# andyburke/bitflood

Hardware: AMD Instinct MI355X
Metric: GiB/s device-resident chunk hashing, 256 KiB chunks, at 1/2/4/8 MI355X (higher is better)
Workload: dtype u32

## Files before the change

### bitflood_amd/_capi.py

```python
from __future__ import annotations

import ctypes
import os
import re

try:
    import torch
except Exception:
    torch = None

_HERE = os.path.dirname(os.path.abspath(__file__))
_REPO = os.path.dirname(_HERE)
LIB_PATH = os.environ.get("LBF_LIB") or os.path.join(_HERE, "lib", "liblbfhash.so")
HEADER_PATH = os.path.join(_REPO, "include", "lbf_hash.h")

LBF_OK = 0
LBF_ERR_INVALID = -1
LBF_ERR_NO_DEVICE = -2
LBF_ERR_HIP = -3
LBF_ERR_NOMEM = -4
LBF_ERR_IO = -5
LBF_HOST_PTR = 0
LBF_DEVICE_PTR = 1

_u8p = ctypes.POINTER(ctypes.c_uint8)
_c = ctypes
_SIGS = {
    "lbf_abi_version": (_c.c_int, []),
    "lbf_last_error": (_c.c_char_p, []),
    "lbf_device_count": (_c.c_int, [_c.POINTER(_c.c_int)]),
    "lbf_ctx_create": (_c.c_int, [_c.c_uint32, _c.POINTER(_c.c_void_p)]),
    "lbf_ctx_destroy": (None, [_c.c_void_p]),
    "lbf_ctx_num_devices": (_c.c_int, [_c.c_void_p]),
    "lbf_ctx_num_workers": (_c.c_int, [_c.c_void_p]),
    "lbf_ctx_worker_info": (_c.c_int, [_c.c_void_p, _c.c_int, _c.POINTER(_c.c_int), _c.POINTER(_c.c_int),
                                       _c.POINTER(_c.c_int), _c.POINTER(_c.c_int)]),
    "lbf_sha1_batch": (_c.c_int, [_c.c_void_p, _c.c_void_p, _c.c_uint64, _c.c_void_p, _c.c_void_p,
                                  _c.c_uint64, _c.c_void_p, _c.c_int]),
    "lbf_verify_batch": (_c.c_int, [_c.c_void_p, _c.c_void_p, _c.c_uint64, _c.c_void_p, _c.c_void_p,
                                    _c.c_uint64, _c.c_void_p, _c.c_void_p, _c.c_int]),
    "lbf_host_register": (_c.c_int, [_c.c_void_p, _c.c_void_p, _c.c_uint64]),
    "lbf_host_unregister": (_c.c_int, [_c.c_void_p, _c.c_void_p]),
    "lbf_ctx_staging_stats": (_c.c_int, [_c.c_void_p, _c.POINTER(_c.c_uint64), _c.POINTER(_c.c_uint64)]),
    "lbf_ctx_b64_stats": (_c.c_int, [_c.c_void_p, _c.POINTER(_c.c_uint64), _c.POINTER(_c.c_uint64)]),
    "lbf_sha1_one": (_c.c_int, [_c.c_void_p, _c.c_void_p, _c.c_uint32, _c.c_void_p]),
    "lbf_verify_encode_b64_batch": (_c.c_int, [_c.c_void_p, _c.c_void_p, _c.c_uint64, _c.c_void_p, _c.c_void_p,
                                               _c.c_uint64, _c.c_void_p, _c.c_void_p, _c.c_void_p, _c.c_uint64,
                                               _c.c_void_p]),
    "lbf_b64_put_length": (_c.c_uint64, [_c.c_uint64]),
    "lbf_b64_verify_batch": (_c.c_int, [_c.c_void_p, _c.c_void_p, _c.c_uint64, _c.c_void_p, _c.c_void_p,
                                        _c.c_uint64, _c.c_void_p, _c.c_void_p, _c.c_void_p, _c.c_uint64,
                                        _c.c_void_p, _c.c_void_p, _c.c_void_p]),
    "lbf_file_ranges": (_c.c_int, [_c.c_void_p, _c.c_char_p, _c.c_void_p, _c.c_void_p, _c.c_uint64,
                                   _c.c_void_p, _c.c_void_p]),
    "lbf_files_ranges": (_c.c_int, [_c.c_void_p, _c.c_void_p, _c.c_uint32, _c.c_void_p, _c.c_void_p, _c.c_void_p,
                                    _c.c_uint64, _c.c_void_p, _c.c_void_p]),
    "lbf_b64_27": (None, [_c.c_void_p, _c.c_char_p]),
    "lbf_b64_27_decode": (_c.c_int, [_c.c_char_p, _c.c_size_t, _c.c_void_p]),
    "lbf_sha1_launch": (_c.c_int, [_c.c_void_p, _c.c_void_p, _c.c_void_p, _c.c_uint64, _c.c_void_p,
                                   _c.c_void_p, _c.c_void_p, _c.c_void_p]),
    "lbf_sha1_uniform_launch": (_c.c_int, [_c.c_void_p, _c.c_uint64, _c.c_uint32, _c.c_uint64,
                                           _c.c_uint64, _c.c_void_p, _c.c_void_p, _c.c_void_p,
                                           _c.c_void_p]),
    "lbf_sha1_state_init": (None, [_c.c_void_p, _c.c_uint64]),
    "lbf_sha1_update_launch": (_c.c_int, [_c.c_void_p, _c.c_uint64, _c.c_void_p, _c.c_void_p, _c.c_void_p,
                                          _c.c_void_p, _c.c_void_p, _c.c_uint64, _c.c_void_p, _c.c_void_p,
                                          _c.c_void_p, _c.c_void_p]),
    "lbf_sha1_update_batch": (_c.c_int, [_c.c_void_p, _c.c_void_p, _c.c_uint64, _c.c_void_p, _c.c_void_p,
                                         _c.c_uint64, _c.c_void_p, _c.c_void_p, _c.c_void_p, _c.c_uint64,
                                         _c.c_void_p, _c.c_void_p, _c.c_void_p]),
    "lbf_b64_state_init": (None, [_c.c_void_p, _c.c_uint64]),
    "lbf_b64_update_launch": (_c.c_int, [_c.c_void_p, _c.c_void_p, _c.c_uint64, _c.c_void_p, _c.c_void_p, _c.c_void_p,
                                         _c.c_void_p, _c.c_void_p, _c.c_uint64, _c.c_void_p, _c.c_void_p, _c.c_void_p,
                                         _c.c_void_p, _c.c_void_p, _c.c_void_p, _c.c_void_p, _c.c_void_p, _c.c_void_p,
                                         _c.c_void_p]),
    "lbf_b64_update_batch": (_c.c_int, [_c.c_void_p, _c.c_void_p, _c.c_void_p, _c.c_uint64, _c.c_void_p, _c.c_void_p,
                                        _c.c_uint64, _c.c_void_p, _c.c_void_p, _c.c_void_p, _c.c_uint64, _c.c_void_p,
                                        _c.c_void_p, _c.c_void_p, _c.c_uint64, _c.c_void_p, _c.c_void_p, _c.c_void_p]),
    "lbf_set_kernel_variant": (_c.c_int, [_c.c_int]),
    "lbf_get_kernel_variant": (_c.c_int, []),
    "lbf_kernel_for": (_c.c_int, [_c.c_uint64]),
    "lbf_fill_synthetic": (_c.c_int, [_c.c_void_p, _c.c_uint64, _c.c_uint64, _c.c_uint64, _c.c_void_p]),
    "lbf_dev_malloc": (_c.c_int, [_c.POINTER(_c.c_void_p), _c.c_uint64]),
    "lbf_dev_free": (_c.c_int, [_c.c_void_p]),
    "lbf_memcpy_h2d": (_c.c_int, [_c.c_void_p, _c.c_void_p, _c.c_uint64]),
    "lbf_memcpy_d2h": (_c.c_int, [_c.c_void_p, _c.c_void_p, _c.c_uint64]),
    "lbf_set_device": (_c.c_int, [_c.c_int]),
    "lbf_device_synchronize": (_c.c_int, []),
    "lbf_stream_create": (_c.c_int, [_c.POINTER(_c.c_void_p)]),
    "lbf_stream_destroy": (_c.c_int, [_c.c_void_p]),
    "lbf_stream_synchronize": (_c.c_int, [_c.c_void_p]),
    "lbf_time_uniform": (_c.c_int, [_c.c_void_p, _c.c_uint64, _c.c_uint32, _c.c_uint64, _c.c_uint64,
                                    _c.c_void_p, _c.c_int, _c.c_void_p, _c.POINTER(_c.c_float)]),
}

_lib = None


class LbfError(RuntimeError):
    def __init__(self, status: int, msg: str):
        super().__init__(f"lbf status {status}: {msg}")
        self.status = status


def header_symbols(path: str = HEADER_PATH) -> list[str]:
    text = open(path).read()
    text = re.sub(r"/\*.*?\*/", "", text, flags=re.S)
    return sorted(set(re.findall(r"\b(lbf_[a-z0-9_]+)\s*\(", text)))


def load() -> ctypes.CDLL:
    global _lib
    if _lib is not None:
        return _lib
    if not os.path.exists(LIB_PATH):
        raise LbfError(LBF_ERR_INVALID,
                       f"{LIB_PATH} is not built; run `python -c 'import __graft_entry__ as g; g.build()'`")
    lib = ctypes.CDLL(LIB_PATH)
    for name, (res, args) in _SIGS.items():
        try:
            fn = getattr(lib, name)
        except AttributeError:
            if "LBF_LIB" in os.environ:
                continue
            raise
        fn.restype = res
        fn.argtypes = args
    _lib = lib
    return lib


def check(rc: int) -> None:
    if rc != LBF_OK:
        msg = load().lbf_last_error()
        raise LbfError(rc, msg.decode() if msg else "")


def device_count() -> int:
    n = ctypes.c_int(0)
    check(load().lbf_device_count(ctypes.byref(n)))
    return n.value
```

### bitflood_amd/csrc/lbf_internal.hpp

```cpp
#pragma once

#include <hip/hip_runtime.h>
#include <stdint.h>

#include <string>

#include "lbf_hash.h"

namespace lbf {

void set_error(const std::string& msg);
int fail(int status, const std::string& msg);
int hip_fail(hipError_t e, const char* what);

#define LBF_HIP_TRY(expr)                                   \
  do {                                                      \
    hipError_t lbf_e_ = (expr);                             \
    if (lbf_e_ != hipSuccess) return ::lbf::hip_fail(lbf_e_, #expr); \
  } while (0)

struct ChunkParams {
  const uint8_t* base;
  const uint64_t* offsets;
  const uint32_t* sizes;
  uint64_t len;
  uint64_t first_chunk;
  uint32_t chunk_size;
  uint32_t n;
  uint8_t* digests;
  const uint8_t* expected;
  uint8_t* verdicts;
};

int check_fits(const void* p, uint64_t bytes, const char* what);

int pick_variant(uint64_t n);
int launch_chunks(const ChunkParams& p, hipStream_t stream);

struct B64Launch {
  const uint8_t* text;
  uint8_t* scratch;
  const uint64_t* text_off;
  const uint64_t* sext_off;
  const uint32_t* text_len;
  uint8_t* out;
  const uint64_t* out_off;
  const uint32_t* cap;
  uint32_t* sizes;
  uint8_t* over;
  uint8_t* redo;
  uint32_t n;
  uint32_t max_text_len;
  uint32_t max_cap;
};
int launch_b64_decode(const B64Launch& b, hipStream_t stream);
int launch_b64_encode(const uint8_t* data, const uint64_t* data_off, const uint32_t* size, uint8_t* text,
                      const uint64_t* text_off, uint32_t n, uint32_t max_size, hipStream_t stream);

struct ExtraVariants {
  bool (*known)(int variant);
  bool (*launch)(int variant, const ChunkParams& p, hipStream_t stream);
};
extern const ExtraVariants* g_extra_variants;

}
```

### bitflood_amd/csrc/sha1_update.hip

```cpp
#include <hip/hip_runtime.h>
#include <stddef.h>

#include "lbf_internal.hpp"
#include "sha1_device.hpp"

namespace lbf {

namespace {

struct UpdateParams {
  uint8_t* states;
  uint64_t n_states;
  const uint32_t* state_of;
  const uint8_t* base;
  const uint64_t* offsets;
  const uint32_t* sizes;
  const uint8_t* final_flags;
  uint32_t n;
  uint8_t* digests;
  const uint8_t* expected;
  uint8_t* verdicts;
};

constexpr uint32_t kStateBytes = 96, kBlockAt = 32;
static_assert(sizeof(lbf_sha1_state) == kStateBytes, "lbf_sha1_state is 96 bytes");
static_assert(offsetof(lbf_sha1_state, buffered) == 20 && offsetof(lbf_sha1_state, total) == 24 &&
                  offsetof(lbf_sha1_state, block) == kBlockAt,
              "lbf_sha1_state layout");

__device__ __forceinline__ void load_block(uint4 (&q)[4], const uint4* src) {
  q[0] = src[0];
  q[1] = src[1];
  q[2] = src[2];
  q[3] = src[3];
}

__device__ __forceinline__ void update_blocks_aligned(Digest& s, const uint8_t* src, uint32_t nblk) {
  if (nblk == 0) return;
  const uint4* q = reinterpret_cast<const uint4*>(src);
  const uint32_t last = nblk - 1;
  uint4 A[4], B[4];
  load_block(A, q);
  load_block(B, q + 4 * (last < 1u ? last : 1u));
  for (uint32_t b = 0; b < nblk; ++b) {
    uint4 C[4] = {A[0], A[1], A[2], A[3]};
    A[0] = B[0]; A[1] = B[1]; A[2] = B[2]; A[3] = B[3];
    const uint32_t nb = b + 2 < last ? b + 2 : last;
    load_block(B, q + 4 * nb);
    uint32_t w[16];
    block_from_vec(w, C[0], C[1], C[2], C[3]);
    compress(s, w);
  }
}

__device__ __forceinline__ void update_blocks_unaligned(Digest& s, const uint8_t* src, uint32_t nblk) {
  for (uint32_t b = 0; b < nblk; ++b) {
    uint32_t w[16];
    load_words_any(w, src + 64ull * b, 64);
#pragma unroll
    for (int k = 0; k < 16; ++k) w[k] = bswap(w[k]);
    compress(s, w);
  }
}

__device__ __forceinline__ void record_block(uint32_t (&w)[16], const uint8_t* blk) {
  const uint4* q = reinterpret_cast<const uint4*>(blk);
  const uint4 q0 = q[0], q1 = q[1], q2 = q[2], q3 = q[3];
  block_from_vec(w, q0, q1, q2, q3);
}

__device__ __forceinline__ void finish64(Digest& s, uint32_t (&w)[16], uint32_t r, uint64_t total) {
#pragma unroll
  for (int k = 0; k < 16; ++k) {
    const int rem = (int)r - 4 * k;
    uint32_t v = w[k];
    if (rem <= 0) v = 0;
    if (rem >= 0 && rem < 4) {
      const uint32_t sh = 8u * (uint32_t)rem;
      v = (v & ~(0xFFFFFFFFu >> sh)) | (0x80000000u >> sh);
    }
    w[k] = v;
  }
  if (r >= 56) {
    compress(s, w);
#pragma unroll
    for (int k = 0; k < 16; ++k) w[k] = 0;
  }
  w[14] = (uint32_t)(total >> 29);
  w[15] = (uint32_t)(total << 3);
  compress(s, w);
}

__global__ void __launch_bounds__(256) sha1_update_kernel(UpdateParams p) {
  const uint32_t i = blockIdx.x * blockDim.x + threadIdx.x;
  if (i >= p.n) return;
  const uint64_t si = p.state_of ? (uint64_t)p.state_of[i] : (uint64_t)i;
  if (si >= p.n_states) return;
  uint8_t* const rec = p.states + kStateBytes * si;
  uint8_t* const blk = rec + kBlockAt;

  const uint4 lo = reinterpret_cast<const uint4*>(rec)[0];
  const uint4 hi = reinterpret_cast<const uint4*>(rec)[1];
  Digest s;
  s.h[0] = lo.x; s.h[1] = lo.y; s.h[2] = lo.z; s.h[3] = lo.w; s.h[4] = hi.x;
  uint32_t buf = hi.y & 63u;
  uint64_t total = (uint64_t)hi.z | ((uint64_t)hi.w << 32);

  const uint8_t* src = p.base + p.offsets[i];
  uint32_t size = p.sizes[i];
  const bool fin = p.final_flags != nullptr && p.final_flags[i] != 0;
  total += size;

  if (buf) {
    const uint32_t room = 64u - buf;
    const uint32_t take = size < room ? size : room;
    for (uint32_t k = 0; k < take; ++k) blk[(buf + k) & 63u] = src[k];
    src += take;
    size -= take;
    buf += take;
    if (buf == 64u) {
      uint32_t w[16];
      record_block(w, blk);
      compress(s, w);
      buf = 0;
    }
  }
  const uint32_t nblk = size >> 6;
  if ((reinterpret_cast<uintptr_t>(src) & 15u) == 0) {
    update_blocks_aligned(s, src, nblk);
  } else {
    update_blocks_unaligned(s, src, nblk);
  }
  src += 64ull * nblk;
  const uint32_t rem = size & 63u;
  for (uint32_t k = 0; k < rem; ++k) blk[(buf + k) & 63u] = src[k];
  buf = (buf + rem) & 63u;

  uint4* const out = reinterpret_cast<uint4*>(rec);
  if (!fin) {
    out[0] = make_uint4(s.h[0], s.h[1], s.h[2], s.h[3]);
    out[1] = make_uint4(s.h[4], buf, (uint32_t)total, (uint32_t)(total >> 32));
    return;
  }

  uint32_t w[16];
  record_block(w, blk);
  finish64(s, w, buf, total);
  uint32_t be[5];
#pragma unroll
  for (int k = 0; k < 5; ++k) be[k] = bswap(s.h[k]);
  if (p.digests) {
    uint32_t* o = reinterpret_cast<uint32_t*>(p.digests + 20ull * i);
#pragma unroll
    for (int k = 0; k < 5; ++k) o[k] = be[k];
  }
  if (p.verdicts) {
    const uint32_t* e = reinterpret_cast<const uint32_t*>(p.expected + 20ull * i);
    uint32_t diff = 0;
#pragma unroll
    for (int k = 0; k < 5; ++k) diff |= be[k] ^ e[k];
    p.verdicts[i] = diff == 0 ? 1 : 0;
  }
  out[0] = make_uint4(kH0, kH1, kH2, kH3);
  out[1] = make_uint4(kH4, 0u, 0u, 0u);
#pragma unroll
  for (int k = 2; k < 6; ++k) out[k] = make_uint4(0u, 0u, 0u, 0u);
}

}

}

using lbf::check_fits;
using lbf::fail;

extern "C" void lbf_sha1_state_init(lbf_sha1_state* states, uint64_t n) {
  if (!states) return;
  for (uint64_t k = 0; k < n; ++k) {
    lbf_sha1_state& s = states[k];
    s.h[0] = lbf::kH0; s.h[1] = lbf::kH1; s.h[2] = lbf::kH2; s.h[3] = lbf::kH3; s.h[4] = lbf::kH4;
    s.buffered = 0;
    s.total = 0;
    for (int j = 0; j < 64; ++j) s.block[j] = 0;
  }
}

extern "C" int lbf_sha1_update_launch(lbf_sha1_state* d_states, uint64_t n_states, const uint32_t* d_state_of,
                                      const uint8_t* d_base, const uint64_t* d_offsets, const uint32_t* d_sizes,
                                      const uint8_t* d_final, uint64_t n, uint8_t* d_digests,
                                      const uint8_t* d_expected, uint8_t* d_verdicts, void* stream) {
  const char* who = "lbf_sha1_update_launch";
  if (n == 0) return LBF_OK;
  if (!d_states || !d_base || !d_offsets || !d_sizes) return fail(LBF_ERR_INVALID, std::string(who) + ": null input");
  if (n > 0xFFFFFFFFull) return fail(LBF_ERR_INVALID, std::string(who) + ": n exceeds 2^32-1 per launch");
  if (d_final && !d_digests && !d_verdicts) return fail(LBF_ERR_INVALID, std::string(who) + ": no output");
  if ((d_verdicts != nullptr) != (d_expected != nullptr))
    return fail(LBF_ERR_INVALID, std::string(who) + ": expected and verdicts go together");
  if ((reinterpret_cast<uintptr_t>(d_digests) & 3u) || (reinterpret_cast<uintptr_t>(d_expected) & 3u))
    return fail(LBF_ERR_INVALID, std::string(who) + ": digest/expected arrays must be 4-byte aligned");
  if (reinterpret_cast<uintptr_t>(d_states) & 15u)
    return fail(LBF_ERR_INVALID, std::string(who) + ": the state array must be 16-byte aligned");
  if (n_states > UINT64_MAX / 96) return fail(LBF_ERR_INVALID, std::string(who) + ": n_states too large");
  if (int rc = check_fits(d_states, 96 * n_states, "lbf_sha1_update_launch: states")) return rc;
  if (int rc = check_fits(d_state_of, 4 * n, "lbf_sha1_update_launch: state_of")) return rc;
  if (int rc = check_fits(d_offsets, 8 * n, "lbf_sha1_update_launch: offsets")) return rc;
  if (int rc = check_fits(d_sizes, 4 * n, "lbf_sha1_update_launch: sizes")) return rc;
  if (int rc = check_fits(d_final, n, "lbf_sha1_update_launch: final")) return rc;
  if (int rc = check_fits(d_digests, 20 * n, "lbf_sha1_update_launch: digests")) return rc;
  if (int rc = check_fits(d_expected, 20 * n, "lbf_sha1_update_launch: expected")) return rc;
  if (int rc = check_fits(d_verdicts, n, "lbf_sha1_update_launch: verdicts")) return rc;
  lbf::UpdateParams p{};
  p.states = reinterpret_cast<uint8_t*>(d_states);
  p.n_states = n_states;
  p.state_of = d_state_of;
  p.base = d_base;
  p.offsets = d_offsets;
  p.sizes = d_sizes;
  p.final_flags = d_final;
  p.n = (uint32_t)n;
  p.digests = d_digests;
  p.expected = d_expected;
  p.verdicts = d_verdicts;
  const uint32_t threads = p.n <= 65536u ? 64u : 256u;
  hipLaunchKernelGGL(lbf::sha1_update_kernel, dim3((p.n + threads - 1) / threads), dim3(threads), 0,
                     (hipStream_t)stream, p);
  LBF_HIP_TRY(hipGetLastError());
  return LBF_OK;
}
```

### bitflood_amd/csrc/update_batch.cpp

```cpp
#include <hip/hip_runtime.h>
#include <string.h>

#include <algorithm>

#include "lbf_host.hpp"
#include "update_plan.hpp"

using namespace lbf;

namespace {

uint64_t up(uint64_t x, uint64_t a) { return (x + a - 1) / a * a; }

int update_scratch(lbf_ctx* ctx, uint64_t need) {
  return grow_scratch(ctx->upd_dev, ctx->upd_cap, need, up(need, 1ull << 20), "lbf_sha1_update_batch");
}

struct UpdateCall {
  lbf_sha1_state* states;
  const uint32_t* state_of;
  const uint8_t* base;
  const uint8_t* final_flags;
  uint8_t* out_digests;
  const uint8_t* expected;
  uint8_t* verdicts;
};

int update_run_launch(lbf_ctx* ctx, hipStream_t st, const UpdateCall& c, const std::vector<UpdateCut>& cuts) {
  const uint64_t m = cuts.size();
  if (m == 0) return LBF_OK;
  std::vector<Run> runs;
  std::vector<uint64_t> dev_off;
  const uint64_t area = update_runs(cuts, runs, dev_off);
  const uint64_t st_b = 96 * m, off_at = st_b, size_at = off_at + 8 * m, exp_at = size_at + 4 * m,
                 fin_at = exp_at + 20 * m, in_bytes = fin_at + m;
  std::vector<uint8_t> in(in_bytes, 0), res(21 * m, 0);
  SyncOnExit sync{st};
  lbf_sha1_state* h_states = reinterpret_cast<lbf_sha1_state*>(in.data());
  uint64_t* h_off = reinterpret_cast<uint64_t*>(in.data() + off_at);
  uint32_t* h_size = reinterpret_cast<uint32_t*>(in.data() + size_at);
  bool any_final = false;
  for (uint64_t k = 0; k < m; ++k) {
    const uint64_t i = cuts[k].piece;
    h_states[k] = c.states[update_state_of(c.state_of, i)];
    h_off[k] = dev_off[k];
    h_size[k] = cuts[k].size;
    if (c.expected) memcpy(in.data() + exp_at + 20 * k, c.expected + 20 * i, 20);
    const bool fin = cuts[k].last && c.final_flags && c.final_flags[i];
    in[fin_at + k] = fin ? 1 : 0;
    any_final |= fin;
  }
  const uint64_t data_b = up(area + 16, 256), in_b = up(in_bytes, 256);
  if (int rc = update_scratch(ctx, data_b + in_b + up(21 * m, 256))) return rc;
  uint8_t* d_data = ctx->upd_dev;
  uint8_t* d_in = d_data + data_b;
  uint8_t* d_res = d_in + in_b;
  for (const Run& r : runs)
    LBF_HIP_TRY(hipMemcpyAsync(d_data + r.dst, c.base + r.src, r.len, hipMemcpyHostToDevice, st));
  LBF_HIP_TRY(hipMemcpyAsync(d_in, in.data(), in.size(), hipMemcpyHostToDevice, st));
  uint8_t* d_dig = d_res;
  uint8_t* d_ver = d_res + 20 * m;
  if (int rc = lbf_sha1_update_launch(reinterpret_cast<lbf_sha1_state*>(d_in), m, nullptr, d_data,
                                      reinterpret_cast<const uint64_t*>(d_in + off_at),
                                      reinterpret_cast<const uint32_t*>(d_in + size_at), d_in + fin_at, m, d_dig,
                                      c.expected ? d_in + exp_at : nullptr, c.expected ? d_ver : nullptr, st))
    return rc;
  LBF_HIP_TRY(hipMemcpyAsync(in.data(), d_in, st_b, hipMemcpyDeviceToHost, st));
  if (any_final) LBF_HIP_TRY(hipMemcpyAsync(res.data(), d_res, res.size(), hipMemcpyDeviceToHost, st));
  LBF_HIP_TRY(hipStreamSynchronize(st));
  for (uint64_t k = 0; k < m; ++k) {
    const uint64_t i = cuts[k].piece;
    c.states[update_state_of(c.state_of, i)] = h_states[k];
    if (!in[fin_at + k]) continue;
    if (c.out_digests) memcpy(c.out_digests + 20 * i, res.data() + 20 * k, 20);
    if (c.verdicts) c.verdicts[i] = res[20 * m + k];
  }
  return LBF_OK;
}

}

extern "C" int lbf_sha1_update_batch(lbf_ctx* ctx, lbf_sha1_state* states, uint64_t n_states, const uint32_t* state_of,
                                     const uint8_t* base, uint64_t base_len, const uint64_t* offsets,
                                     const uint32_t* sizes, const uint8_t* final_flags, uint64_t n,
                                     uint8_t* out_digests, const uint8_t* expected, uint8_t* verdicts) {
  const char* who = "lbf_sha1_update_batch";
  if (!ctx) return fail(LBF_ERR_INVALID, "null context");
  if (n == 0) return LBF_OK;
  if (!states || !base || !offsets || !sizes) return fail(LBF_ERR_INVALID, std::string(who) + ": null argument");
  if (n > 0x7FFFFFFFull) return fail(LBF_ERR_INVALID, std::string(who) + ": n too large");
  if ((verdicts != nullptr) != (expected != nullptr))
    return fail(LBF_ERR_INVALID, std::string(who) + ": expected and verdicts go together");
  return guarded([&]() -> int {
    std::string why;
    const uint64_t bad = update_check(states, n_states, state_of, base_len, offsets, sizes, n, why);
    if (bad != kNoPiece) return fail(LBF_ERR_INVALID, std::string(who) + ": piece " + std::to_string(bad) + " " + why);
    const std::vector<std::vector<UpdateCut>> launches = update_launches(offsets, sizes, n, ctx->update_bytes);
    const UpdateCall call{states, state_of, base, final_flags, out_digests, expected, verdicts};
    std::lock_guard<std::mutex> lock(ctx->mu);
    KeepCurrentDevice keep;
    Worker& w = ctx->workers[0];
    LBF_HIP_TRY(hipSetDevice(w.device));
    hipStream_t st = w.dev[0].stream;
    for (const std::vector<UpdateCut>& cuts : launches)
      if (int rc = update_run_launch(ctx, st, call, cuts)) return rc;
    return (int)LBF_OK;
  });
}
```

### bitflood_amd/hashing.py

```python
from __future__ import annotations

import ctypes
import os

import numpy as np

from . import _capi
from ._capi import LBF_DEVICE_PTR, LBF_HOST_PTR, LbfError, check, load

DIGEST = 20
_EMPTY = (ctypes.c_uint8 * 1)()


STATE_DTYPE = np.dtype({"names": ["h", "buffered", "total", "block"],
                        "formats": [(np.uint32, 5), np.uint32, np.uint64, (np.uint8, 64)],
                        "offsets": [0, 20, 24, 32], "itemsize": 96})


def new_states(n: int) -> np.ndarray:
    states = np.zeros(int(n), dtype=STATE_DTYPE)
    if states.size:
        load().lbf_sha1_state_init(states.ctypes.data, states.size)
    return states

# ... 252 lines not shown

    def verify_files(self, paths, file_of, offsets, sizes, expected) -> np.ndarray:
        return self._files_call(paths, file_of, offsets, sizes, expected).astype(bool)

    def verify_b64(self, text, text_offsets, text_lens, expected_sizes, expected, out=None, out_offsets=None):
        buf = _as_u8(text)
        toff = np.ascontiguousarray(text_offsets, dtype=np.uint64)
        tlen = np.ascontiguousarray(text_lens, dtype=np.uint32)
        esz = np.ascontiguousarray(expected_sizes, dtype=np.uint32)
        exp = np.ascontiguousarray(expected, dtype=np.uint8).reshape(-1, DIGEST)
        n = toff.size
        if not (tlen.size == esz.size == exp.shape[0] == n):
            raise ValueError("text_offsets, text_lens, expected_sizes and expected differ in length")
        ver = np.zeros(n, dtype=np.uint8)
        sizes = np.zeros(n, dtype=np.uint32)
        if n == 0:
            return ver.astype(bool), sizes
        ooff = None
        if out is not None:
            if not (isinstance(out, np.ndarray) and out.dtype == np.uint8 and out.flags.c_contiguous):
                raise ValueError("out must be a C-contiguous uint8 array")
            ooff = np.ascontiguousarray(out_offsets, dtype=np.uint64)
            if ooff.size != n:
                raise ValueError("out_offsets differs in length")
        base = buf.ctypes.data if buf.size else ctypes.addressof(_EMPTY)
        check(self._lib.lbf_b64_verify_batch(self._h, base, buf.size, toff.ctypes.data, tlen.ctypes.data, n,
                                             esz.ctypes.data, exp.ctypes.data,
                                             None if out is None else out.ctypes.data,
                                             0 if out is None else out.size,
                                             None if ooff is None else ooff.ctypes.data, sizes.ctypes.data,
                                             ver.ctypes.data))
        return ver.astype(bool), sizes

    def verify_encode_b64(self, data, offsets, sizes, expected):
        buf = _as_u8(data)
        offs = np.ascontiguousarray(offsets, dtype=np.uint64)
        sz = np.ascontiguousarray(sizes, dtype=np.uint32)
        exp = np.ascontiguousarray(expected, dtype=np.uint8).reshape(-1, DIGEST)
        n = offs.size
        if not (sz.size == exp.shape[0] == n):
            raise ValueError("offsets, sizes and expected differ in length")
        ver = np.zeros(n, dtype=np.uint8)
        if n == 0:
            return ver.astype(bool), []
        lens = [int(self._lib.lbf_b64_put_length(int(s))) for s in sz]
        toff = np.zeros(n, dtype=np.uint64)
        pos = 0
        for i, tl in enumerate(lens):
            toff[i] = pos
            pos += (tl + 15) // 16 * 16
        text = np.zeros(max(pos, 1), dtype=np.uint8)
        base = buf.ctypes.data if buf.size else ctypes.addressof(_EMPTY)
        check(self._lib.lbf_verify_encode_b64_batch(self._h, base, buf.size, offs.ctypes.data, sz.ctypes.data, n,
                                                    exp.ctypes.data, ver.ctypes.data, text.ctypes.data, text.size,
                                                    toff.ctypes.data))
        return ver.astype(bool), [text[int(toff[i]):int(toff[i]) + lens[i]].tobytes() for i in range(n)]

    def sha1(self, data) -> bytes:
        buf = _as_u8(data)
        out = (ctypes.c_uint8 * DIGEST)()
        base = buf.ctypes.data if buf.size else ctypes.addressof(_EMPTY)
        check(self._lib.lbf_sha1_one(self._h, base, buf.size, out))
        return bytes(out)

    def base64_encode(self, data) -> str:
        return b64_27(self.sha1(data))

    def encode_buffer(self, data, chunk_size: int) -> list[str]:
        buf = _as_u8(data)
        offs, sizes = chunk_table(buf.size, chunk_size)
        return [b64_27(bytes(d)) for d in self.hash_chunks(buf, offs, sizes)]


class DeviceBuffer:
    def __init__(self, nbytes: int):
        self.nbytes = int(nbytes)
        p = ctypes.c_void_p()
        check(load().lbf_dev_malloc(ctypes.byref(p), self.nbytes))
        self.ptr = p.value

    def free(self):
        if self.ptr:
            check(load().lbf_dev_free(self.ptr))
            self.ptr = None

    def _range(self, offset: int, nbytes: int, what: str):
        if not self.ptr:
            raise ValueError(f"{what}: buffer already freed")
        if offset < 0 or nbytes < 0 or offset + nbytes > self.nbytes:
            raise ValueError(f"{what}: [{offset}, {offset + nbytes}) outside the {self.nbytes}-byte buffer")

    def upload(self, host: np.ndarray, offset: int = 0):
        host = np.ascontiguousarray(host)
        self._range(offset, host.nbytes, "upload")
        check(load().lbf_memcpy_h2d(self.ptr + offset, host.ctypes.data, host.nbytes))

    def download(self, nbytes: int | None = None, offset: int = 0, dtype=np.uint8) -> np.ndarray:
        nbytes = self.nbytes - offset if nbytes is None else nbytes
        self._range(offset, nbytes, "download")
        out = np.empty(nbytes, dtype=np.uint8)
        check(load().lbf_memcpy_d2h(out.ctypes.data, self.ptr + offset, nbytes))
        return out.view(dtype)

    def download_into(self, out: np.ndarray, offset: int = 0) -> None:
        if not isinstance(out, np.ndarray) or not out.flags.c_contiguous:
            raise ValueError("download_into: out must be a C-contiguous numpy array")
        self._range(offset, out.nbytes, "download_into")
        if out.nbytes:
            check(load().lbf_memcpy_d2h(out.ctypes.data, self.ptr + offset, out.nbytes))

    def fill_synthetic(self, seed: int, start: int = 0, nbytes: int | None = None, stream=None, offset: int = 0):
        nbytes = self.nbytes - offset if nbytes is None else nbytes
        self._range(offset, nbytes, "fill_synthetic")
        check(load().lbf_fill_synthetic(self.ptr + offset, nbytes, seed, start, stream))


def uniform_launch(base: DeviceBuffer | int, length: int, chunk_size: int, first: int, n: int,
                   digests: DeviceBuffer | int | None, expected=None, verdicts=None, stream=None):
    p = lambda x: None if x is None else (x.ptr if isinstance(x, DeviceBuffer) else x)
    check(load().lbf_sha1_uniform_launch(p(base), length, chunk_size, first, n, p(digests), p(expected),
                                         p(verdicts), stream))


def batch_launch(base, offsets, sizes, n, digests, expected=None, verdicts=None, stream=None):
    p = lambda x: None if x is None else (x.ptr if isinstance(x, DeviceBuffer) else x)
    check(load().lbf_sha1_launch(p(base), p(offsets), p(sizes), n, p(digests), p(expected), p(verdicts),
                                 stream))


def update_launch(states, n_states, state_of, base, offsets, sizes, final, n, digests, expected=None, verdicts=None,
                  stream=None):
    p = lambda x: None if x is None else (x.ptr if isinstance(x, DeviceBuffer) else x)
    check(load().lbf_sha1_update_launch(p(states), n_states, p(state_of), p(base), p(offsets), p(sizes), p(final), n,
                                        p(digests), p(expected), p(verdicts), stream))


def b64_update_launch(b64_states, sha_states, n_states, state_of, text, text_offsets, text_lens, final, n, out,
                      out_offsets, caps, out_sizes, digests, expected, verdicts, piece_offsets, piece_sizes,
                      stream=None):
    p = lambda x: None if x is None else (x.ptr if isinstance(x, DeviceBuffer) else x)
    check(load().lbf_b64_update_launch(p(b64_states), p(sha_states), n_states, p(state_of), p(text), p(text_offsets),
                                       p(text_lens), p(final), n, p(out), p(out_offsets), p(caps), p(out_sizes),
                                       p(digests), p(expected), p(verdicts), p(piece_offsets), p(piece_sizes), stream))


def synchronize():
    check(load().lbf_device_synchronize())


def set_kernel_variant(v: int):
    check(load().lbf_set_kernel_variant(v))


__all__ = ["ChunkHasher", "DeviceBuffer", "LbfError", "b64_27", "b64_27_decode", "chunk_table",
           "uniform_launch", "batch_launch", "update_launch", "STATE_DTYPE", "new_states",
           "B64_STATE_DTYPE", "new_b64_states", "b64_update_launch", "synchronize", "set_kernel_variant", "LBF_DEVICE_PTR",
           "_capi"]
```

### include/lbf_hash.h

```cpp
#ifndef LBF_HASH_H_
#define LBF_HASH_H_

#include <stddef.h>
#include <stdint.h>

#ifdef __cplusplus
extern "C" {
#endif

#define LBF_ABI_VERSION 1
#define LBF_DIGEST_BYTES 20
#define LBF_B64_CHARS 27

typedef enum lbf_status {
  LBF_OK = 0,
  LBF_ERR_INVALID = -1,
  LBF_ERR_NO_DEVICE = -2,
  LBF_ERR_HIP = -3,
  LBF_ERR_NOMEM = -4,
  LBF_ERR_IO = -5
} lbf_status;

#define LBF_HOST_PTR 0
#define LBF_DEVICE_PTR 1

typedef struct lbf_ctx lbf_ctx;

int lbf_abi_version(void);
const char* lbf_last_error(void);
int lbf_device_count(int* out_count);
int lbf_ctx_create(uint32_t device_mask, lbf_ctx** out_ctx);
void lbf_ctx_destroy(lbf_ctx* ctx);
int lbf_ctx_num_devices(const lbf_ctx* ctx);
int lbf_ctx_num_workers(const lbf_ctx* ctx);
int lbf_ctx_worker_info(const lbf_ctx* ctx, int worker, int* device, int* numa_node, int* staging_node,
                        int* bound_cpus);

int lbf_sha1_batch(lbf_ctx* ctx, const uint8_t* base, uint64_t base_len,
                   const uint64_t* offsets, const uint32_t* sizes, uint64_t n,
                   uint8_t* out_digests, int flags);

int lbf_verify_batch(lbf_ctx* ctx, const uint8_t* base, uint64_t base_len,
                     const uint64_t* offsets, const uint32_t* sizes, uint64_t n,
                     const uint8_t* expected, uint8_t* verdicts, int flags);

int lbf_host_register(lbf_ctx* ctx, const void* ptr, uint64_t len);
int lbf_host_unregister(lbf_ctx* ctx, const void* ptr);
int lbf_ctx_staging_stats(lbf_ctx* ctx, uint64_t* staged_bytes, uint64_t* direct_bytes);

int lbf_file_ranges(lbf_ctx* ctx, const char* path, const uint64_t* offsets, const uint32_t* sizes,
                    uint64_t n, const uint8_t* expected, uint8_t* out);
int lbf_files_ranges(lbf_ctx* ctx, const char* const* paths, uint32_t n_files, const uint32_t* file_of,
                     const uint64_t* offsets, const uint32_t* sizes, uint64_t n, const uint8_t* expected,
                     uint8_t* out);

int lbf_b64_verify_batch(lbf_ctx* ctx, const char* text, uint64_t text_len, const uint64_t* text_offsets,
                         const uint32_t* text_lens, uint64_t n, const uint32_t* expected_sizes,
                         const uint8_t* expected, uint8_t* out, uint64_t out_len, const uint64_t* out_offsets,
                         uint32_t* out_sizes, uint8_t* verdicts);

int lbf_verify_encode_b64_batch(lbf_ctx* ctx, const uint8_t* data, uint64_t data_len, const uint64_t* offsets,
                                const uint32_t* sizes, uint64_t n, const uint8_t* expected, uint8_t* verdicts,
                                char* text, uint64_t text_len, const uint64_t* text_offsets);
int lbf_ctx_b64_stats(lbf_ctx* ctx, uint64_t* one_pass_chunks, uint64_t* general_chunks);
uint64_t lbf_b64_put_length(uint64_t size);

int lbf_sha1_one(lbf_ctx* ctx, const uint8_t* data, uint32_t size, uint8_t out_digest[20]);

void lbf_b64_27(const uint8_t digest[20], char out[28]);
int lbf_b64_27_decode(const char* in, size_t len, uint8_t out_digest[20]);

int lbf_sha1_launch(const uint8_t* d_base, const uint64_t* d_offsets,
                    const uint32_t* d_sizes, uint64_t n, uint8_t* d_digests,
                    const uint8_t* d_expected, uint8_t* d_verdicts, void* stream);
int lbf_sha1_uniform_launch(const uint8_t* d_base, uint64_t len, uint32_t chunk_size,
                            uint64_t first_chunk, uint64_t n, uint8_t* d_digests,
                            const uint8_t* d_expected, uint8_t* d_verdicts, void* stream);
int lbf_set_kernel_variant(int variant);
int lbf_get_kernel_variant(void);
int lbf_kernel_for(uint64_t n_chunks);

typedef struct lbf_sha1_state {
  uint32_t h[5];
  uint32_t buffered;
  uint64_t total;
  uint8_t  block[64];
} lbf_sha1_state;
void lbf_sha1_state_init(lbf_sha1_state* states, uint64_t n);

int lbf_sha1_update_launch(lbf_sha1_state* d_states, uint64_t n_states, const uint32_t* d_state_of,
                           const uint8_t* d_base, const uint64_t* d_offsets, const uint32_t* d_sizes,
                           const uint8_t* d_final, uint64_t n, uint8_t* d_digests,
                           const uint8_t* d_expected, uint8_t* d_verdicts, void* stream);
int lbf_sha1_update_batch(lbf_ctx* ctx, lbf_sha1_state* states, uint64_t n_states, const uint32_t* state_of,
                          const uint8_t* base, uint64_t base_len, const uint64_t* offsets,
                          const uint32_t* sizes, const uint8_t* final_flags, uint64_t n,
                          uint8_t* out_digests, const uint8_t* expected, uint8_t* verdicts);

typedef struct lbf_b64_state {
  uint64_t decoded;
  uint32_t carry;
  uint8_t  ncarry;
  uint8_t  ended;
  uint16_t zero;
} lbf_b64_state;
void lbf_b64_state_init(lbf_b64_state* states, uint64_t n);

int lbf_b64_update_launch(lbf_b64_state* d_b64_states, lbf_sha1_state* d_sha_states, uint64_t n_states,
                          const uint32_t* d_state_of, const char* d_text, const uint64_t* d_text_offsets,
                          const uint32_t* d_text_lens, const uint8_t* d_final, uint64_t n, uint8_t* d_out,
                          const uint64_t* d_out_offsets, const uint32_t* d_caps, uint32_t* d_out_sizes,
                          uint8_t* d_digests, const uint8_t* d_expected, uint8_t* d_verdicts,
                          uint64_t* d_piece_offsets, uint32_t* d_piece_sizes, void* stream);
int lbf_b64_update_batch(lbf_ctx* ctx, lbf_b64_state* b64_states, lbf_sha1_state* sha_states, uint64_t n_states,
                         const uint32_t* state_of, const char* text, uint64_t text_len,
                         const uint64_t* text_offsets, const uint32_t* text_lens, const uint8_t* final_flags,
                         uint64_t n, const uint32_t* expected_sizes, const uint8_t* expected, uint8_t* out,
                         uint64_t out_len, const uint64_t* out_offsets, uint32_t* out_sizes, uint8_t* verdicts);

int lbf_fill_synthetic(uint8_t* d_buf, uint64_t len, uint64_t seed, uint64_t start, void* stream);

int lbf_dev_malloc(void** out_ptr, uint64_t bytes);
int lbf_dev_free(void* ptr);
int lbf_memcpy_h2d(void* dst, const void* src, uint64_t bytes);
int lbf_memcpy_d2h(void* dst, const void* src, uint64_t bytes);
int lbf_set_device(int device);
int lbf_device_synchronize(void);
int lbf_stream_create(void** out_stream);
int lbf_stream_destroy(void* stream);
int lbf_stream_synchronize(void* stream);
int lbf_time_uniform(const uint8_t* d_base, uint64_t len, uint32_t chunk_size,
                     uint64_t first_chunk, uint64_t n, uint8_t* d_digests, int reps,
                     void* stream, float* out_ms_per_launch);

#ifdef __cplusplus
}
#endif

#endif
```

Baseline: 1273.

## Add producer/consumer wave-specialized kernel for SHA-1 streaming update path

Adds a new SHA-1 update kernel in which two producer waves DMA 64-byte blocks of each piece into an LDS ring while a consumer wave runs the compression steps. This reuses the pc4 chunk kernel's scheduling for the stateful update API. An automatic heuristic picks it for small piece counts with large pieces, and a setter exposes a manual override. It targets per-lane memory latency in the update path, at the cost of 96 KiB of LDS per block and extra complexity.

```diff
diff --git a/bitflood_amd/_capi.py b/bitflood_amd/_capi.py
--- a/bitflood_amd/_capi.py
+++ b/bitflood_amd/_capi.py
@@ -79,6 +79,8 @@
                                         _c.c_void_p, _c.c_void_p, _c.c_uint64, _c.c_void_p, _c.c_void_p, _c.c_void_p]),
     "lbf_set_kernel_variant": (_c.c_int, [_c.c_int]),
     "lbf_get_kernel_variant": (_c.c_int, []),
+    "lbf_set_update_kernel": (_c.c_int, [_c.c_int]),
+    "lbf_get_update_kernel": (_c.c_int, []),
     "lbf_kernel_for": (_c.c_int, [_c.c_uint64]),
     "lbf_fill_synthetic": (_c.c_int, [_c.c_void_p, _c.c_uint64, _c.c_uint64, _c.c_uint64, _c.c_void_p]),
     "lbf_dev_malloc": (_c.c_int, [_c.POINTER(_c.c_void_p), _c.c_uint64]),
diff --git a/bitflood_amd/csrc/lbf_internal.hpp b/bitflood_amd/csrc/lbf_internal.hpp
--- a/bitflood_amd/csrc/lbf_internal.hpp
+++ b/bitflood_amd/csrc/lbf_internal.hpp
@@ -37,6 +37,25 @@
 int pick_variant(uint64_t n);
 int launch_chunks(const ChunkParams& p, hipStream_t stream);
 
+struct UpdateParams {
+  uint8_t* states;
+  uint64_t n_states;
+  const uint32_t* state_of;
+  const uint8_t* base;
+  const uint64_t* offsets;
+  const uint32_t* sizes;
+  const uint8_t* final_flags;
+  uint32_t n;
+  uint8_t* digests;
+  const uint8_t* expected;
+  uint8_t* verdicts;
+};
+int launch_update_pc(const UpdateParams& p, hipStream_t stream);
+int update_launch_sized(lbf_sha1_state* d_states, uint64_t n_states, const uint32_t* d_state_of, const uint8_t* d_base,
+                        const uint64_t* d_offsets, const uint32_t* d_sizes, const uint8_t* d_final, uint64_t n,
+                        uint8_t* d_digests, const uint8_t* d_expected, uint8_t* d_verdicts, void* stream,
+                        uint32_t max_piece);
+
 struct B64Launch {
   const uint8_t* text;
   uint8_t* scratch;
diff --git a/bitflood_amd/csrc/sha1_update.hip b/bitflood_amd/csrc/sha1_update.hip
--- a/bitflood_amd/csrc/sha1_update.hip
+++ b/bitflood_amd/csrc/sha1_update.hip
@@ -1,26 +1,17 @@
 #include <hip/hip_runtime.h>
 #include <stddef.h>
 
+#include <atomic>
+
 #include "lbf_internal.hpp"
 #include "sha1_device.hpp"
+#include "update_pc_plan.hpp"
 
 namespace lbf {
 
 namespace {
 
-struct UpdateParams {
-  uint8_t* states;
-  uint64_t n_states;
-  const uint32_t* state_of;
-  const uint8_t* base;
-  const uint64_t* offsets;
-  const uint32_t* sizes;
-  const uint8_t* final_flags;
-  uint32_t n;
-  uint8_t* digests;
-  const uint8_t* expected;
-  uint8_t* verdicts;
-};
+std::atomic<int> g_update_kernel{0};
 
 constexpr uint32_t kStateBytes = 96, kBlockAt = 32;
 static_assert(sizeof(lbf_sha1_state) == kStateBytes, "lbf_sha1_state is 96 bytes");
@@ -185,10 +176,27 @@
   }
 }
 
+extern "C" int lbf_set_update_kernel(int kernel) {
+  if (kernel < 0 || kernel > 2)
+    return fail(LBF_ERR_INVALID, "unknown update kernel (0 automatic, 1 lane form, 2 producer/consumer form)");
+  lbf::g_update_kernel.store(kernel);
+  return LBF_OK;
+}
+
+extern "C" int lbf_get_update_kernel(void) { return lbf::g_update_kernel.load(); }
+
 extern "C" int lbf_sha1_update_launch(lbf_sha1_state* d_states, uint64_t n_states, const uint32_t* d_state_of,
                                       const uint8_t* d_base, const uint64_t* d_offsets, const uint32_t* d_sizes,
                                       const uint8_t* d_final, uint64_t n, uint8_t* d_digests,
                                       const uint8_t* d_expected, uint8_t* d_verdicts, void* stream) {
+  return lbf::update_launch_sized(d_states, n_states, d_state_of, d_base, d_offsets, d_sizes, d_final, n, d_digests,
+                                  d_expected, d_verdicts, stream, lbf::kUpdatePieceUnknown);
+}
+
+int lbf::update_launch_sized(lbf_sha1_state* d_states, uint64_t n_states, const uint32_t* d_state_of,
+                             const uint8_t* d_base, const uint64_t* d_offsets, const uint32_t* d_sizes,
+                             const uint8_t* d_final, uint64_t n, uint8_t* d_digests, const uint8_t* d_expected,
+                             uint8_t* d_verdicts, void* stream, uint32_t max_piece) {
   const char* who = "lbf_sha1_update_launch";
   if (n == 0) return LBF_OK;
   if (!d_states || !d_base || !d_offsets || !d_sizes) return fail(LBF_ERR_INVALID, std::string(who) + ": null input");
@@ -221,6 +229,8 @@
   p.digests = d_digests;
   p.expected = d_expected;
   p.verdicts = d_verdicts;
+  if (lbf::update_kernel_choice(lbf::g_update_kernel.load(), n, max_piece) == 2)
+    return lbf::launch_update_pc(p, (hipStream_t)stream);
   const uint32_t threads = p.n <= 65536u ? 64u : 256u;
   hipLaunchKernelGGL(lbf::sha1_update_kernel, dim3((p.n + threads - 1) / threads), dim3(threads), 0,
                      (hipStream_t)stream, p);
diff --git a/bitflood_amd/csrc/sha1_update_pc.hip b/bitflood_amd/csrc/sha1_update_pc.hip
--- /dev/null
+++ b/bitflood_amd/csrc/sha1_update_pc.hip
@@ -0,0 +1,228 @@
+#include <hip/hip_runtime.h>
+#include <stddef.h>
+
+#include <mutex>
+#include <type_traits>
+
+#define LBF_PLAN_FN __host__ __device__ inline
+#include "kern_pc.hpp"
+#include "update_pc_plan.hpp"
+
+namespace lbf {
+
+namespace {
+
+constexpr uint32_t kStateBytes = 96, kBlockAt = 32;
+static_assert(sizeof(lbf_sha1_state) == kStateBytes, "lbf_sha1_state is 96 bytes");
+static_assert(offsetof(lbf_sha1_state, buffered) == 20 && offsetof(lbf_sha1_state, total) == 24 &&
+                  offsetof(lbf_sha1_state, block) == kBlockAt,
+              "lbf_sha1_state layout");
+
+constexpr int kUpdatePcLdsBytes = kPc4LdsBytes + 16;
+static_assert(kPc4LdsBytes == 96 * 1024, "pc4's ring and raw slots are 96 KiB");
+
+struct PieceInfo {
+  UpdatePcPlan plan;
+  uint8_t* rec;
+  const uint8_t* src;
+  const uint8_t* mid;
+  uint32_t buf;
+  bool active, fin, aligned;
+};
+
+__device__ __forceinline__ PieceInfo piece_info(const UpdateParams& p, uint32_t i) {
+  PieceInfo c{};
+  c.src = c.mid = reinterpret_cast<const uint8_t*>(g_pc_dummy);
+  if (i >= p.n) return c;
+  const uint64_t si = p.state_of ? (uint64_t)p.state_of[i] : (uint64_t)i;
+  if (si >= p.n_states) return c;
+  c.active = true;
+  c.rec = p.states + kStateBytes * si;
+  const uint4 hi = reinterpret_cast<const uint4*>(c.rec)[1];
+  c.buf = hi.y & 63u;
+  c.fin = p.final_flags != nullptr && p.final_flags[i] != 0;
+  c.plan = update_pc_plan(hi.y, (uint64_t)hi.z | ((uint64_t)hi.w << 32), p.sizes[i], c.fin);
+  c.src = p.base + p.offsets[i];
+  c.mid = c.src + c.plan.take;
+  c.aligned = (reinterpret_cast<uintptr_t>(c.mid) & 15u) == 0;
+  return c;
+}
+
+__device__ __forceinline__ void piece_dma(const PieceInfo& c, uint32_t step, uint32_t raw_lds, uint32_t slot) {
+  const bool ok = c.aligned && update_pc_source(c.plan, step) == kPcFromPiece;
+  const uint8_t* src = ok ? c.mid + 64ull * (step - c.plan.head) : reinterpret_cast<const uint8_t*>(g_pc_dummy);
+  const uint32_t base = raw_lds + slot * (kPcRawU4 * 16);
+#pragma unroll
+  for (int j = 0; j < 4; ++j) dma16(src + 16 * j, base + j * (kPcLanes * 16));
+}
+
+template <bool kStep0>
+__device__ __forceinline__ void piece_block(uint32_t (&w)[16], const uint4* raw, const PieceInfo& c,
+                                            const uint32_t (&head)[16], uint32_t step) {
+  const uint32_t from = update_pc_source(c.plan, step);
+  if (from == kPcFromPiece) {
+    if (c.aligned) {
+      block_from_vec(w, raw[0], raw[kPcLanes], raw[2 * kPcLanes], raw[3 * kPcLanes]);
+    } else {
+      load_words_any(w, c.mid + 64ull * (step - c.plan.head), 64);
+#pragma unroll
+      for (int k = 0; k < 16; ++k) w[k] = bswap(w[k]);
+    }
+  } else if (kStep0 && from == kPcFromRecord) {
+#pragma unroll
+    for (int k = 0; k < 16; ++k) w[k] = head[k];
+  } else if (from == kPcFinal0 || from == kPcFinal1) {
+    const uint4* q = reinterpret_cast<const uint4*>(c.rec + kBlockAt);
+    const uint4 q0 = q[0], q1 = q[1], q2 = q[2], q3 = q[3];
+    block_from_vec(w, q0, q1, q2, q3);
+    uint32_t r = c.plan.buffered;
+    asm volatile("" : "+v"(r));
+#pragma unroll
+    for (int k = 0; k < 16; ++k) w[k] = update_pc_final_word(w[k], k, r, c.plan.total, from);
+  } else {
+#pragma unroll
+    for (int k = 0; k < 16; ++k) w[k] = 0;
+  }
+}
+
+__device__ __forceinline__ void piece_head_and_tail(const PieceInfo& c, uint32_t (&head)[16]) {
+#pragma unroll
+  for (int k = 0; k < 16; ++k) head[k] = 0;
+  if (!c.active) return;
+  uint8_t* const blk = c.rec + kBlockAt;
+  for (uint32_t k = 0; k < c.plan.take; ++k) blk[(c.buf + k) & 63u] = c.src[k];
+  if (c.plan.head) {
+    const uint4* q = reinterpret_cast<const uint4*>(blk);
+    const uint4 q0 = q[0], q1 = q[1], q2 = q[2], q3 = q[3];
+    block_from_vec(head, q0, q1, q2, q3);
+  }
+  const uint8_t* tail = c.mid + 64ull * c.plan.nfull;
+  for (uint32_t k = 0; k < c.plan.rem; ++k) blk[k & 63u] = tail[k];
+}
+
+__device__ __forceinline__ void write_piece_result(const UpdateParams& p, uint32_t i, const PieceInfo& c,
+                                                   const Digest& s) {
+  uint4* const out = reinterpret_cast<uint4*>(c.rec);
+  if (!c.fin) {
+    out[0] = make_uint4(s.h[0], s.h[1], s.h[2], s.h[3]);
+    out[1] = make_uint4(s.h[4], c.plan.buffered, (uint32_t)c.plan.total, (uint32_t)(c.plan.total >> 32));
+    return;
+  }
+  ChunkParams r{};
+  r.digests = p.digests;
+  r.expected = p.expected;
+  r.verdicts = p.verdicts;
+  write_result(r, i, s);
+  out[0] = make_uint4(kH0, kH1, kH2, kH3);
+  out[1] = make_uint4(kH4, 0u, 0u, 0u);
+#pragma unroll
+  for (int k = 2; k < 6; ++k) out[k] = make_uint4(0u, 0u, 0u, 0u);
+}
+
+__global__ void __launch_bounds__(192) sha1_update_pc_kernel(UpdateParams p) {
+  extern __shared__ __attribute__((aligned(16))) uint4 ring[];
+  const int lane = threadIdx.x & 63;
+  const int wave = __builtin_amdgcn_readfirstlane(threadIdx.x >> 6);
+  const uint32_t i = blockIdx.x * kPcLanes + lane;
+  const PieceInfo c = piece_info(p, i);
+  uint32_t* const shared_steps = reinterpret_cast<uint32_t*>(ring + kPc4LdsBytes / 16);
+
+  if (wave != 0) {
+    const uint32_t X = wave - 1;
+    uint32_t head[16];
+    if (X == 0) {
+      piece_head_and_tail(c, head);
+      asm volatile("s_waitcnt vmcnt(0)" ::: "memory");
+    } else {
+#pragma unroll
+      for (int k = 0; k < 16; ++k) head[k] = 0;
+    }
+    PC4_SYNC();
+    const uint32_t nsteps = __builtin_amdgcn_readfirstlane(*shared_steps);
+    uint4* raw = ring + kPc4Ring * kPcSlotU4 + X * (kP2Raw * kPcRawU4);
+    const uint32_t raw_lds = (uint32_t)reinterpret_cast<uintptr_t>(raw);
+    piece_dma(c, X, raw_lds, 0);
+    piece_dma(c, X + 2, raw_lds, 1);
+    uint32_t w[16];
+    auto first_half = [&](uint32_t step, auto step0) {
+      const uint32_t j = (step - X) >> 1;
+      asm volatile("s_waitcnt vmcnt(4)" ::: "memory");
+      piece_block<decltype(step0)::value>(w, raw + (j & 1u) * kPcRawU4 + lane, c, head, step);
+      asm volatile("s_waitcnt lgkmcnt(0)" ::: "memory");
+      piece_dma(c, step + 4, raw_lds, j & 1u);
+      pc4_store_half<2, 0>(w, ring, step, lane);
+    };
+    for (uint32_t b = 0; b < nsteps; ++b) {
+      if (b == 0 && X == 0) {
+        first_half(0, std::true_type{});
+        pc4_store_half<2, 1>(w, ring, 0, lane);
+      }
+      const uint32_t fin = b + 1;
+      if ((fin & 1u) == X && fin < nsteps) {
+        if (b == 0) first_half(fin, std::false_type{});
+        pc4_store_half<2, 1>(w, ring, fin, lane);
+      }
+      const uint32_t start = b + 2;
+      if ((start & 1u) == X && start < nsteps) first_half(start, std::false_type{});
+      PC4_SYNC();
+    }
+    asm volatile("s_waitcnt vmcnt(0)" ::: "memory");
+  } else {
+    Digest s;
+    s.init();
+    if (c.active) {
+      const uint4 lo = reinterpret_cast<const uint4*>(c.rec)[0];
+      const uint4 hi = reinterpret_cast<const uint4*>(c.rec)[1];
+      s.h[0] = lo.x; s.h[1] = lo.y; s.h[2] = lo.z; s.h[3] = lo.w; s.h[4] = hi.x;
+    }
+    asm volatile("" : "+v"(s.h[0]), "+v"(s.h[1]), "+v"(s.h[2]), "+v"(s.h[3]), "+v"(s.h[4]));
+    const uint32_t my_max = __builtin_amdgcn_readfirstlane(wave_max(c.plan.nsteps));
+    if (lane == 0) *shared_steps = my_max;
+    PC4_SYNC();
+    const uint32_t nsteps = __builtin_amdgcn_readfirstlane(*shared_steps);
+    Pc4Sched<2> A, B;
+    const uint32_t min_steps = __builtin_amdgcn_readfirstlane(wave_min(c.active ? c.plan.nsteps : 0xFFFFFFFFu));
+    if (nsteps > 0) {
+      PC4_SYNC();
+      A.load_all(Pc4Sched<2>::col(ring, 0, lane));
+      __builtin_amdgcn_s_waitcnt(0xc07f);
+    }
+    uint32_t k = 0;
+    constexpr int kUnroll = 8;
+    const uint32_t fast_end = __builtin_amdgcn_readfirstlane(nsteps ? min(min_steps, nsteps - 1) : 0u);
+    for (; k + kUnroll <= fast_end; k += kUnroll) {
+#pragma unroll
+      for (int j = 0; j < kUnroll; j += 2) {
+        pc4_step(s, A, B, Pc4Sched<2>::col(ring, (j + 1) % 4, lane), true, true);
+        pc4_barrier(s);
+        pc4_step(s, B, A, Pc4Sched<2>::col(ring, (j + 2) % 4, lane), true, true);
+        pc4_barrier(s);
+      }
+    }
+    for (; k < nsteps; k += 2) {
+      pc4_step(s, A, B, Pc4Sched<2>::col(ring, (k + 1) % kPc4Ring, lane), k < c.plan.nsteps, k < min_steps);
+      if (k + 1 >= nsteps) break;
+      pc4_barrier(s);
+      pc4_step(s, B, A, Pc4Sched<2>::col(ring, (k + 2) % kPc4Ring, lane), k + 1 < c.plan.nsteps, k + 1 < min_steps);
+      if (k + 2 >= nsteps) break;
+      pc4_barrier(s);
+    }
+    if (c.active) write_piece_result(p, i, c, s);
+  }
+}
+
+}
+
+int launch_update_pc(const UpdateParams& p, hipStream_t stream) {
+  static std::once_flag once;
+  std::call_once(once, [] {
+    (void)hipFuncSetAttribute(reinterpret_cast<const void*>(&sha1_update_pc_kernel),
+                              hipFuncAttributeMaxDynamicSharedMemorySize, kUpdatePcLdsBytes);
+  });
+  hipLaunchKernelGGL(sha1_update_pc_kernel, dim3((p.n + kPcLanes - 1) / kPcLanes), dim3(192), kUpdatePcLdsBytes,
+                     stream, p);
+  LBF_HIP_TRY(hipGetLastError());
+  return LBF_OK;
+}
+
+}
diff --git a/bitflood_amd/csrc/update_batch.cpp b/bitflood_amd/csrc/update_batch.cpp
--- a/bitflood_amd/csrc/update_batch.cpp
+++ b/bitflood_amd/csrc/update_batch.cpp
@@ -40,8 +40,10 @@
   uint64_t* h_off = reinterpret_cast<uint64_t*>(in.data() + off_at);
   uint32_t* h_size = reinterpret_cast<uint32_t*>(in.data() + size_at);
   bool any_final = false;
+  uint32_t max_piece = 0;
   for (uint64_t k = 0; k < m; ++k) {
     const uint64_t i = cuts[k].piece;
+    max_piece = std::max(max_piece, cuts[k].size);
     h_states[k] = c.states[update_state_of(c.state_of, i)];
     h_off[k] = dev_off[k];
     h_size[k] = cuts[k].size;
@@ -60,10 +62,10 @@
   LBF_HIP_TRY(hipMemcpyAsync(d_in, in.data(), in.size(), hipMemcpyHostToDevice, st));
   uint8_t* d_dig = d_res;
   uint8_t* d_ver = d_res + 20 * m;
-  if (int rc = lbf_sha1_update_launch(reinterpret_cast<lbf_sha1_state*>(d_in), m, nullptr, d_data,
-                                      reinterpret_cast<const uint64_t*>(d_in + off_at),
-                                      reinterpret_cast<const uint32_t*>(d_in + size_at), d_in + fin_at, m, d_dig,
-                                      c.expected ? d_in + exp_at : nullptr, c.expected ? d_ver : nullptr, st))
+  if (int rc = update_launch_sized(reinterpret_cast<lbf_sha1_state*>(d_in), m, nullptr, d_data,
+                                   reinterpret_cast<const uint64_t*>(d_in + off_at),
+                                   reinterpret_cast<const uint32_t*>(d_in + size_at), d_in + fin_at, m, d_dig,
+                                   c.expected ? d_in + exp_at : nullptr, c.expected ? d_ver : nullptr, st, max_piece))
     return rc;
   LBF_HIP_TRY(hipMemcpyAsync(in.data(), d_in, st_b, hipMemcpyDeviceToHost, st));
   if (any_final) LBF_HIP_TRY(hipMemcpyAsync(res.data(), d_res, res.size(), hipMemcpyDeviceToHost, st));
diff --git a/bitflood_amd/csrc/update_pc_plan.hpp b/bitflood_amd/csrc/update_pc_plan.hpp
--- /dev/null
+++ b/bitflood_amd/csrc/update_pc_plan.hpp
@@ -0,0 +1,79 @@
+#pragma once
+
+#include <stdint.h>
+
+#ifndef LBF_PLAN_FN
+#define LBF_PLAN_FN inline
+#endif
+
+namespace lbf {
+
+struct UpdatePcPlan {
+  uint32_t take;
+  uint32_t head;
+  uint32_t nfull;
+  uint32_t rem;
+  uint32_t buffered;
+  uint32_t finals;
+  uint32_t nsteps;
+  uint64_t total;
+};
+
+enum UpdatePcSource : uint32_t {
+  kPcFromRecord = 0,
+  kPcFromPiece = 1,
+  kPcFinal0 = 2,
+  kPcFinal1 = 3,
+  kPcPastEnd = 4,
+};
+
+LBF_PLAN_FN UpdatePcPlan update_pc_plan(uint32_t buffered, uint64_t total, uint32_t size, bool final_piece) {
+  UpdatePcPlan p{};
+  const uint32_t buf = buffered & 63u;
+  if (buf) {
+    const uint32_t room = 64u - buf;
+    p.take = size < room ? size : room;
+  }
+  p.head = (buf != 0 && buf + p.take == 64u) ? 1u : 0u;
+  const uint32_t left = size - p.take;
+  p.nfull = left >> 6;
+  p.rem = left & 63u;
+  p.buffered = (buf != 0 && !p.head) ? buf + p.take : p.rem;
+  p.total = total + size;
+  p.finals = final_piece ? (p.buffered >= 56u ? 2u : 1u) : 0u;
+  p.nsteps = p.head + p.nfull + p.finals;
+  return p;
+}
+
+LBF_PLAN_FN uint32_t update_pc_source(const UpdatePcPlan& p, uint32_t step) {
+  if (step < p.head) return kPcFromRecord;
+  if (step - p.head < p.nfull) return kPcFromPiece;
+  if (step >= p.nsteps) return kPcPastEnd;
+  return step - p.head - p.nfull == 0 ? kPcFinal0 : kPcFinal1;
+}
+
+LBF_PLAN_FN uint32_t update_pc_len_hi(uint64_t total) { return (uint32_t)(total >> 29); }
+LBF_PLAN_FN uint32_t update_pc_len_lo(uint64_t total) { return (uint32_t)(total << 3); }
+
+LBF_PLAN_FN uint32_t update_pc_final_word(uint32_t be, int k, uint32_t r, uint64_t total, uint32_t source) {
+  const bool second = source == kPcFinal1;
+  if (k >= 14 && (second || r < 56u)) return k == 14 ? update_pc_len_hi(total) : update_pc_len_lo(total);
+  if (second) return 0u;
+  const int left = (int)r - 4 * k;
+  if (left >= 4) return be;
+  if (left < 0) return 0u;
+  const uint32_t sh = 8u * (uint32_t)left;
+  return (left ? be & ~(0xFFFFFFFFu >> sh) : 0u) | (0x80000000u >> sh);
+}
+
+constexpr uint64_t kUpdatePcMaxPieces = 16384;
+constexpr uint32_t kUpdatePcMinPiece = 512;
+constexpr uint32_t kUpdatePieceUnknown = 0xFFFFFFFFu;
+
+LBF_PLAN_FN int update_kernel_choice(int setting, uint64_t n, uint32_t max_piece) {
+  if (setting == 1 || n > kUpdatePcMaxPieces) return 1;
+  if (setting == 2) return 2;
+  return max_piece < kUpdatePcMinPiece ? 1 : 2;
+}
+
+}
diff --git a/bitflood_amd/hashing.py b/bitflood_amd/hashing.py
--- a/bitflood_amd/hashing.py
+++ b/bitflood_amd/hashing.py
@@ -428,7 +428,16 @@
     check(load().lbf_set_kernel_variant(v))
 
 
+def set_update_kernel(k: int):
+    check(load().lbf_set_update_kernel(k))
+
+
+def get_update_kernel() -> int:
+    return load().lbf_get_update_kernel()
+
+
 __all__ = ["ChunkHasher", "DeviceBuffer", "LbfError", "b64_27", "b64_27_decode", "chunk_table",
            "uniform_launch", "batch_launch", "update_launch", "STATE_DTYPE", "new_states",
-           "B64_STATE_DTYPE", "new_b64_states", "b64_update_launch", "synchronize", "set_kernel_variant", "LBF_DEVICE_PTR",
+           "B64_STATE_DTYPE", "new_b64_states", "b64_update_launch", "synchronize", "set_kernel_variant",
+           "set_update_kernel", "get_update_kernel", "LBF_DEVICE_PTR",
            "_capi"]
diff --git a/include/lbf_hash.h b/include/lbf_hash.h
--- a/include/lbf_hash.h
+++ b/include/lbf_hash.h
@@ -92,6 +92,8 @@
                            const uint8_t* d_base, const uint64_t* d_offsets, const uint32_t* d_sizes,
                            const uint8_t* d_final, uint64_t n, uint8_t* d_digests,
                            const uint8_t* d_expected, uint8_t* d_verdicts, void* stream);
+int lbf_set_update_kernel(int kernel);
+int lbf_get_update_kernel(void);
 int lbf_sha1_update_batch(lbf_ctx* ctx, lbf_sha1_state* states, uint64_t n_states, const uint32_t* state_of,
                           const uint8_t* base, uint64_t base_len, const uint64_t* offsets,
                           const uint32_t* sizes, const uint8_t* final_flags, uint64_t n,
```

Result: no change. 1272 (-0.0%).
